# wtaylor17/ImageCFGen-Pytorch

Hardware: AMD Instinct MI355X
Metric: ALI training images/sec (E+G+D step), MorphoMNIST bs=512/GPU (higher is better)
Workload: dtype f32; 1 GPU; image_scms/mnist.py ALI iteration (EG step + 2 D steps + diagnostics), MorphoMNIST 28x28x1 synthetic, bs=512/GPU, fp32 MFMA, mode=stepper+hipgraph; global_batch=512, parallelism=dp1

## Files before the change

imagecfgen-pytorch_amd/ali_hip/_lib.py:

```python
import ctypes
import os
from ctypes import POINTER, Structure, c_char_p, c_double, c_float, c_int32, c_int64, c_size_t, c_uint64, c_void_p

_HERE = os.path.dirname(os.path.abspath(__file__))
LIB_PATH = os.path.join(_HERE, "libali_hip.so")


class AliHipUnavailable(RuntimeError):
    pass


class AliConvGeom(Structure):
    _fields_ = [(n, c_int32) for n in ("B", "H", "W", "C", "P", "Q", "K", "R", "S", "stride", "pad")]


class AliEpilogue(Structure):
    _fields_ = [("bias", c_void_p), ("act", c_int32), ("slope", c_float), ("mask", c_void_p), ("mask_ld", c_int32),
                ("dact_y", c_void_p), ("dact", c_int32), ("dslope", c_float),
                ("bn_part", c_void_p), ("bn_mode", c_int32), ("bn_groups", c_int32), ("bn_stat_mask", c_void_p),
                ("bn_mask_ld", c_int32), ("bn_x", c_void_p), ("bn_mean", c_void_p), ("bn_invstd", c_void_p),
                ("bn_mask_in", c_void_p), ("bn_mask_pre", c_void_p), ("mfma_f16", c_int32),
                ("in16", c_void_p), ("w16", c_void_p), ("out16", c_void_p),
                ("tile_order", c_void_p), ("tile_order_n", c_int32), ("in_ld", c_int32), ("out_ld", c_int32),
                ("in_ch_live", c_int32), ("bn_slots", c_int32), ("dact_y16", c_void_p)]
# ... 183 lines not shown
    "ali_add_i64_multi": (c_int32, [c_int32, POINTER(c_void_p), POINTER(c_int64), c_void_p]),
    "ali_assemble_planes": (c_int32, [c_void_p, c_void_p, POINTER(c_void_p), c_int32, c_void_p, c_int32, c_void_p,
                                      c_int32, c_int32, c_int32, c_int32, c_void_p, c_int32, c_void_p]),
    "ali_spect_post": (c_int32, [c_void_p, c_int32, c_int32, c_int32, c_void_p, c_void_p, c_float, c_void_p, c_void_p]),
    "ali_plane_table_grad": (c_int32, [c_void_p, c_int32, c_int32, c_void_p, c_int32, c_int32, c_void_p, c_int32, c_int32,
                                       c_int32, c_int32, c_int32, c_int32, c_void_p, c_void_p, c_void_p]),
    "ali_col2im": (c_int32, [c_void_p, c_int32, c_void_p, c_void_p] + [c_int32] * 12 + [c_float, c_void_p]),
    "ali_tconv_scatter_ok": (c_int32, [c_int32] * 5),
    "ali_tconv_scatter_wgrad_ws": (c_int64, [c_int32] * 7),
    "ali_tconv_scatter_wgrad": (c_int32, [c_void_p, c_void_p, c_int32, c_void_p, c_int64, c_int64] + [c_int32] * 10
                                + [c_void_p, c_size_t, c_void_p]),
    "ali_tconv_scatter": (c_int32, [c_void_p] * 4 + [c_int32] * 13 + [c_float, c_void_p]),
    "ali_tconv_scatter_plan": (c_int32, [c_int32] * 13 + [POINTER(c_int64)]),
    "ali_tconv1_fwd": (c_int32, [c_void_p, c_void_p, c_void_p, c_void_p] + [c_int32] * 9 + [c_float, c_void_p, c_int32,
                                                                                            c_void_p]),
    "ali_tconv1_dgrad": (c_int32, [c_void_p, c_int32, c_void_p, c_void_p, c_int32, c_float, c_void_p] + [c_int32] * 7
                         + [c_void_p]),
    "ali_tconv1_wgrad": (c_int32, [c_void_p, c_void_p, c_int32, c_int32, c_void_p, c_int64, c_int64, c_int64]
                         + [c_int32] * 7 + [c_void_p, c_size_t, c_void_p]),
    "ali_tconv1_route": (c_int32, [c_int32] * 9 + [c_size_t]),
    "ali_ssim_fwd": (c_int32, [c_void_p, c_void_p, c_int64, c_int32, c_int32, c_void_p, c_int32, c_float, c_float,
                               c_void_p, c_void_p, c_void_p, c_void_p, c_void_p, c_size_t, c_void_p]),
    "ali_ssim_bwd": (c_int32, [c_void_p, c_void_p, c_void_p, c_void_p, c_void_p, c_void_p, c_int64, c_int32, c_int32,
                               c_void_p, c_int32, c_void_p, c_void_p]),
    "ali_gl_init": (c_int32, [c_void_p, c_int32, c_int32, c_int32, c_int32, c_void_p, c_void_p, c_float, c_float, c_void_p,
                              c_void_p, c_int32, c_uint64, c_void_p, c_uint64, c_void_p, c_void_p, c_void_p]),
    "ali_gl_ola": (c_int32, [c_void_p, c_void_p, c_int32, c_int32, c_int32, c_int32, c_int32, c_int32, c_int64, c_int32,
                             c_void_p, c_int32, c_void_p, c_void_p]),
    "ali_gl_phase": (c_int32, [c_void_p, c_void_p, c_void_p, c_float, c_int64, c_int32, c_void_p, c_void_p]),
    "ali_gl_check": (c_int32, [c_int32, c_int32, c_int32, c_int32, c_int64]),
    "ali_last_error": (c_char_p, []),
    "ali_head_fwd": (c_int32, [c_void_p, c_int32, c_void_p, c_void_p, c_void_p, c_int32, c_int32, c_void_p]),
    "ali_head_wgrad": (c_int32, [c_void_p, c_int32, c_void_p, c_void_p, c_void_p, c_int32, c_int32, c_void_p]),
    "ali_copy_multi": (c_int32, [c_int32, POINTER(c_void_p), POINTER(c_void_p), POINTER(c_int64), c_void_p]),
    "ali_version": (c_int32, []),
    "ali_reload_tuning": (None, []),
}

_lib = None
_load_error = None


def load():
    global _lib, _load_error
    if _lib is not None:
        return _lib
    if not os.path.exists(LIB_PATH):
        _load_error = f"{LIB_PATH} not found: build it with `python __graft_entry__.py build` (hipcc, gfx950)"
        raise AliHipUnavailable(_load_error)
    try:
        lib = ctypes.CDLL(LIB_PATH)
    except OSError as e:
        _load_error = f"cannot load {LIB_PATH}: {e}"
        raise AliHipUnavailable(_load_error)
    for name, (res, args) in SIGNATURES.items():
        fn = getattr(lib, name)
        fn.restype = res
        fn.argtypes = args
    _lib = lib
    return lib


def check(rc, what):
    if rc != 0:
        msg = load().ali_last_error()
        raise RuntimeError(f"{what} failed (rc={rc}): {msg.decode() if msg else ''}")
# ... 1 lines not shown
```

imagecfgen-pytorch_amd/ali_hip/chain.py:

```python
import weakref
from collections import namedtuple
from typing import List, Optional

import torch
import torch.nn as nn

from . import dropout as _dropout
from . import ops
from .ops import ACT_LEAKY, ACT_NONE, ACT_TANH


def _pad4(c: int) -> int:
    return (c + 3) // 4 * 4


class Stage:
    __slots__ = ("kind", "mod", "act", "slope", "pre", "pattern", "has_drop", "drop_p", "bn", "unflat", "index", "hw")

    def __init__(self, kind, mod, pre, index):
        self.kind, self.mod, self.pre, self.index = kind, mod, pre, index
        self.act, self.slope, self.unflat = ACT_NONE, 0.0, None
        self.hw = None
        self.pattern = [k for k, _ in pre]
        self.has_drop = "drop" in self.pattern
# ... 603 lines not shown
        if st.kind == "flat":
            resolve_flat(st, (B, H, W, Cp), c_log)
        sv.in_shape, sv.out_shape = (B, H, W, Cp), _out_shape(st, B, H, W, Cp)
        sv.geom, sv.route = _geom(st, sv.in_shape, sv.out_shape), route(st, sv.in_shape, c_log)
        sv.mask = folded if folded is not None else early
        if sv.mask is None and st.has_drop and training:
            sv.mask = _dropout.next_mask(B, c_log, st.drop_p, cur.device, Cp, lane=lane)
        sv.t = _pre_ops(st, sv, bn_fwd and (bn_fwd[0], bn_fwd[3]), folded is not None or (si == 0 and first_mask_applied),
                        groups)
        K = sv.out_shape[3]
        out_ld, jmask = 0, None
        if nxt is None and join is not None:
            joint, joff, jm = join
            if sv.out_shape[1:3] != (1, 1) or joint.shape[0] != B or not join_ok(plan):
                raise ValueError("chain_forward(join=...): the last stage must be a plain conv GEMM onto a 1x1 map")
            out_ld = joint.shape[1]
            sv.y = joint[:, joff:joff + K].unflatten(1, (1, 1, K))
            jmask = None if jm is None else jm[:, joff:joff + K]
        else:
            sv.y = (alloc(("y", si), sv.out_shape) if alloc is not None
                    else torch.empty(sv.out_shape, dtype=torch.float32, device=cur.device))
        folded, early, bn_fwd = _for_next_stage(nxt, sv, groups, lane) if nxt is not None else (None, None, None)
        yield from _launch_fwd(plan, st, sv, folded, bn_fwd, out_ld, jmask, alloc)
        if save:
            saved.append(sv)
        cur, c_log = sv.y, K
    return cur, saved


def wgrad_geoms(plan: ChainPlan, saved):
    return [sv.geom for sv in saved if sv.route.wgrad[0] != "tconv1"]


def _param_grads(st: Stage, sv, g_pre, ld: int, grads, grad_dst, fold):
    m, g = st.mod, sv.geom
    B, H, W, Cp = sv.in_shape
    _, P, Q, K = sv.out_shape
    c_in = sv.c_log
    path, db_path = sv.route.wgrad if fold is None else sv.route.wgrad_fold
    fused_db = None
    if db_path == "unflat":
        Cc, hh, ww = st.unflat
        db = ops.colsum(B, hh * ww * Cc, hh * ww * Cc, g_pre).reshape(hh * ww, Cc).t().reshape(-1)
        grads[id(m.bias)] = grad_dst[id(m.bias)].copy_(db) if id(m.bias) in grad_dst else db
    elif db_path == "fused":
        fused_db = grad_dst.get(id(m.bias))
        if fused_db is None:
            fused_db = torch.empty(K, dtype=torch.float32, device=g_pre.device)
        grads[id(m.bias)] = fused_db
    elif db_path == "colsum":
        grads[id(m.bias)] = ops.colsum(B * P * Q, K, K, g_pre, out=grad_dst.get(id(m.bias)))
    dw = grads[id(m.weight)] = grad_dst[id(m.weight)] if id(m.weight) in grad_dst else torch.empty_like(m.weight)
    if path == "flat_repack":
        O, I, T = m.out_features, m.in_features, H * W
        tmp = torch.empty(O, I, device=dw.device)
        ops.conv_bwd_weight(g, sv.t, g_pre, tmp, I, O, I, 1, 0)
        ops.pack_weights(tmp, dw, O, I // T, T, T, I, 1, I // T)
        return
    if st.kind == "flat":
        ops.conv_bwd_weight(g, sv.t, g_pre, dw, c_in, K, dw.stride(0), H * W, 1, db=fused_db, dy_ld=ld, defer=fold)
        return
    R, S = m.kernel_size if st.kind != "linear" else (1, 1)
    if path == "convT_scatter" and sv.t.is_contiguous() and g_pre.is_contiguous() and dw.stride(2) == S * dw.stride(3):
        if ops.tconv_scatter_wgrad(sv.t, g_pre, 1, dw, dw.stride(0), dw.stride(3), B, H, W, Cp, P, Q, R, S, m.stride[0],
                                   m.padding[0]) is not None:
            return
    if path == "head":
        ops.head_wgrad(sv.t.reshape(B, Cp)[:, :c_in], g_pre.reshape(B), dw.reshape(-1), db=fused_db)
    elif path == "first_direct":
        ops.tconv1_wgrad(g_pre, sv.t, Cp, c_in, dw, c_in * R * S, 1, R * S, B, P, Q, K, R, S, m.padding[0])
    elif path == "conv":
        ops.conv_bwd_weight(g, sv.t, g_pre, dw, c_in, K, dw.stride(0), dw.stride(1), dw.stride(3), db=fused_db,
                            dy_ld=ld, defer=fold)
    elif path == "tconv1":
        ops.tconv1_wgrad(sv.t, g_pre, 1, 1, dw, R * S, 1, 0, B, H, W, Cp, R, S, m.padding[0])
    elif path in ("convT", "convT_scatter"):
        ops.conv_bwd_weight(g, g_pre, sv.t, dw, K, c_in, dw.stride(0), dw.stride(1), dw.stride(3), defer=fold)
    elif path == "linear":
        ops.conv_bwd_weight(g, sv.t, g_pre, dw, m.in_features, m.out_features, m.in_features, 1, 0, defer=fold)
    else:
        (O, I), (Cc, hh, ww) = m.weight.shape, st.unflat
        tmp = torch.empty(O, I, device=dw.device)
        ops.conv_bwd_weight(g, sv.t, g_pre, tmp, I, O, I, 1, 0)
        ops.pack_weights(tmp, dw, Cc, hh * ww, I, I, I, Cc * I, 1)


def _plane_grads(plan: ChainPlan, st: Stage, sv, g_pre, gx_planes):
    m, NP = st.mod, len(gx_planes)
    B, H, W, Cp = sv.in_shape
    _, P, Q, K = sv.out_shape
    R, S = m.kernel_size
    form = sv.route.planes
    if form is None or (form == "scatter" and not (1 <= NP <= 8 and NP * R * S <= 128)):
        return None
    planes = torch.empty(B, H, W, NP, dtype=torch.float32, device=g_pre.device)
    if form == "direct":
        wd = plan.packed(st, "dgrad", Cp)
        for j, c in enumerate(gx_planes):
            ops.tconv1_fwd(g_pre, wd[c], None, planes[..., j], B, P, Q, K, R, S, m.padding[0], NP, ACT_NONE, 0.0,
                           rowscale=None if sv.mask is None else sv.mask[:, c])
        return planes
    wd = plan.packed(st, ("scatter_dgrad", tuple(gx_planes)), Cp)
    if ops.tconv_scatter_ok(K, NP, R, S, m.stride[0]) and g_pre.is_contiguous():
        ops.tconv_scatter(g_pre, wd, None, planes, B, P, Q, K, H, W, NP, NP, R, S, m.stride[0], m.padding[0])
    else:
        contrib = torch.empty(B, P, Q, NP * R * S, dtype=torch.float32, device=g_pre.device)
        ops.conv_fwd(ops.geom(B, P, Q, K, P, Q, NP * R * S, 1, 1, 1, 0), g_pre, wd, contrib, ops.epilogue())
        yield
        ops.col2im(contrib, NP * R * S, None, planes, B, P, Q, H, W, NP, NP, R, S, m.stride[0], m.padding[0])
    if sv.mask is not None:
        cols = torch.cat([sv.mask[:, c:c + 1] for c in gx_planes], dim=1)
        planes = planes * cols.reshape(B, 1, 1, -1)
    return planes


def _data_grad(plan: ChainPlan, st: Stage, sv, g_pre, ld: int, pact, pslope, want: bool, need_params: bool, grads,
               grad_dst):
    m, g, bn, rt = st.mod, sv.geom, sv.bn, sv.route
    B, H, W, Cp = sv.in_shape
    dact_y = sv.x_in if pact != ACT_NONE else None
    gt = torch.empty(sv.in_shape, dtype=torch.float32, device=g_pre.device)
    bn_red = None
    if bn is None:
        ep = ops.epilogue(mask=sv.mask, dact_y=dact_y, dact=pact, dslope=pslope)
    else:
        mask_in = sv.mask if sv.pattern == ["drop", "bn"] else None
        mask_pre = sv.mask if sv.pattern == ["bn", "drop"] else None
        slots = ops.conv_mtiles(g, 0 if rt.dgrad == "convT" else 1)[0] if rt.bn_reduce else 0
        if slots > 0:
            bn_red = (torch.empty(2 * Cp * slots, dtype=torch.float32, device=g_pre.device), slots)
            ep = ops.epilogue(bn_bwd=(bn_red[0], sv.x_in, sv.bn_stats[0], sv.bn_stats[1], mask_in, mask_pre, slots))
        else:
            ep = ops.epilogue()
    if rt.dgrad == "tconv1" and bn is None and sv.mask is None:
        ops.tconv1_dgrad(g_pre, 1, plan.packed(st, "fwd", Cp), dact_y, pact, pslope, gt, B, H, W, Cp, m.kernel_size[0],
                         m.kernel_size[1], m.padding[0])
    elif st.kind == "convT":
        ops.conv_fwd(g, g_pre, plan.packed(st, "dgrad", Cp), gt, ep, live=(None, sv.c_log))
        yield
    else:
        wc = H * W * Cp if rt.dgrad == "flat_gemm" else Cp
        ops.conv_bwd_data(g, g_pre, plan.packed(st, "dgrad", wc), gt, ep, in_ld=ld,
                          live=(wc if rt.dgrad == "flat_gemm" else sv.c_log, None))
        yield
    if bn is None:
        return gt
    use_batch = sv.training or bn.running_mean is None
    slope = pslope if pact == ACT_LEAKY else -1.0
    out = dict(want_gx=want, out_dgamma=grad_dst.get(id(bn.weight)) if need_params else None,
               out_dbeta=grad_dst.get(id(bn.bias)) if need_params else None)
    if bn_red is not None:
        dgam, dbet, gprev = ops.bn_bwd_from_partials(bn_red[0], bn_red[1], sv.x_in, gt, mask_in, mask_pre, sv.bn_stats,
                                                     bn.weight.detach(), B, H * W, Cp, use_batch, slope, **out)
    else:
        dgam, dbet, gprev = ops.bn_bwd(sv.x_in, gt, mask_in, mask_pre, sv.bn_stats, bn.weight.detach(), B, H * W, Cp,
                                       use_batch, slope, **out)
    if need_params:
        grads[id(bn.weight)], grads[id(bn.bias)] = dgam, dbet
    if pact == ACT_TANH and gprev is not None:
        gprev = ops.act_bwd(gprev, sv.x_in, ACT_TANH, 0.0)
    return gprev


def chain_backward_gen(plan: ChainPlan, saved, gy: torch.Tensor, c_log_in: int, need_gx: bool, need_params: bool = True,
                       grad_dst=None, gx_planes=None, gy_ld: int = 0, gy_pre: bool = False, in_act=None, fold=None):
    grads = {}
    grad_dst = grad_dst or {}
    n = len(plan.stages)
    last = plan.stages[-1]
    assert saved[0].c_log == c_log_in, "chain_backward: c_log_in differs from the forward pass's"
    if gy_ld:
        if not (gy_pre or last.act == ACT_NONE) or not join_ok(plan):
            raise ValueError("chain_backward(gy_ld=...): needs join_ok(plan) and a pre-activation gradient")
        g_pre = gy
    else:
        gy = gy.contiguous()
        g_pre = gy if (gy_pre or last.act == ACT_NONE) else ops.act_bwd(gy, saved[-1].y, last.act, last.slope)
    for i in range(n - 1, -1, -1):
        st, sv = plan.stages[i], saved[i]
        assert not isinstance(sv.bn_stats, list), "grouped forward state: backpropagate slice_saved(saved, g, groups)"
        ld = gy_ld if i == n - 1 else 0
        if need_params:
            _param_grads(st, sv, g_pre, ld, grads, grad_dst, fold)
        if i > 0:
            g_pre = yield from _data_grad(plan, st, sv, g_pre, ld, plan.stages[i - 1].act, plan.stages[i - 1].slope, True,
                                          need_params, grads, grad_dst)
    gx = (yield from _plane_grads(plan, st, sv, g_pre, gx_planes)) if gx_planes is not None else None
    if gx is None and (need_gx or sv.bn is not None):
        gx = yield from _data_grad(plan, st, sv, g_pre, ld, *(in_act or (ACT_NONE, 0.0)), need_gx, need_params, grads,
                                   grad_dst)
    return gx, grads


def _plain_stack(plan: ChainPlan, what: str):
    for st in plan.stages:
        if st.pre or st.kind not in ("conv", "flat") or st.act not in (ACT_NONE, ACT_LEAKY):
            raise NotImplementedError(f"ali_hip.chain.{what}: needs a stack of Conv2d / Flatten + Linear stages with "
                                      f"LeakyReLU or no activation and nothing in front of them (stage {st.index}: "
                                      f"{st.kind}, pre-ops {st.pattern}, activation {st.act})")


def saved_rows(saved, lo: int, hi: int):
    out = []
    for sv in saved:
        assert sv.bn is None and sv.bn_stats is None, "saved_rows: BatchNorm statistics couple the rows of a batch"
        s2 = _Saved()
        s2.x_in, s2.t, s2.y = sv.x_in[lo:hi], sv.t[lo:hi], sv.y[lo:hi]
        s2.mask = None if sv.mask is None else sv.mask[lo:hi]
        s2.bn, s2.bn_stats, s2.pattern, s2.training, s2.route, s2.c_log = None, None, sv.pattern, sv.training, sv.route, sv.c_log
        s2.in_shape, s2.out_shape = (hi - lo,) + tuple(sv.in_shape[1:]), (hi - lo,) + tuple(sv.out_shape[1:])
        g = sv.geom
        s2.geom = ops.geom(hi - lo, g.H, g.W, g.C, g.P, g.Q, g.K, g.R, g.S, g.stride, g.pad)
        out.append(s2)
    return out


def chain_backward_keep_gen(plan: ChainPlan, saved, gy: torch.Tensor, c_log_in: int, need_gx: bool = True,
                            gx_planes=None, first_rows=None):
    _plain_stack(plan, "chain_backward_keep")
# ... 120 lines not shown
```

imagecfgen-pytorch_amd/ali_hip/ops.py:

```python
import collections
import ctypes
from ctypes import byref, c_void_p

import numpy as np
import torch

from . import _lib
from ._lib import ACT_LEAKY, ACT_NONE, ACT_TANH, AliConvGeom, AliEpilogue

_WS = {}
_WS_BYTES = 256 << 20


def set_workspace_bytes(n: int):
    global _WS_BYTES
    _WS_BYTES = int(n)
    _WS.clear()


def workspace(device, slot: int = 0) -> torch.Tensor:
    key = (device.type, device.index if device.index is not None else torch.cuda.current_device(), slot)
    ws = _WS.get(key)
    if ws is None or ws.numel() < _WS_BYTES:
        ws = torch.zeros(_WS_BYTES, dtype=torch.uint8, device=device)
# ... 670 lines not shown
def _flush_packs():
    jobs = _PACK_BATCH
    if not jobs:
        return
    _launch_packs(jobs)
    jobs.clear()


def pack_weights(src, dst, N, T, C, Cpad, s_n, s_tap, s_c):
    _chk(src, "src"), _chk(dst, "dst")
    if _PACK_BATCH is not None:
        if any(j[1].data_ptr() == src.data_ptr() for j in _PACK_BATCH):
            _flush_packs()
        _PACK_BATCH.append((src, dst, N, T, C, Cpad, s_n, s_tap, s_c))
        return dst
    _launch_packs([(src, dst, N, T, C, Cpad, s_n, s_tap, s_c)])
    return dst


def head_fwd(x2d, w, bias, y):
    B, C = x2d.shape
    _lib.check(_lib.load().ali_head_fwd(_ptr(x2d), x2d.stride(0), _chk(w, "w"), _opt(bias, "bias"), _chk(y, "y"), B, C,
                                        _stream()), "ali_head_fwd")
    return y


def head_wgrad(x2d, g, dw, db=None):
    B, C = x2d.shape
    _lib.check(_lib.load().ali_head_wgrad(_ptr(x2d), x2d.stride(0), _chk(g, "g"), _chk(dw, "dw"), _opt(db, "db"), B, C,
                                          _stream()), "ali_head_wgrad")
    return dw


def copy_multi(pairs):
    fast = []
    for dst, src in pairs:
        if (dst.is_cuda and src.is_cuda and dst.device == src.device and dst.dtype == src.dtype and dst.shape == src.shape
                and dst.is_contiguous() and src.is_contiguous() and dst.element_size() % 4 == 0 and dst.numel() > 0):
            fast.append((dst, src))
        else:
            dst.copy_(src)
    if fast:
        n = len(fast)
        srcs = (c_void_p * n)(*[s_.data_ptr() for _, s_ in fast])
        dsts = (c_void_p * n)(*[d_.data_ptr() for d_, _ in fast])
        sizes = (ctypes.c_int64 * n)(*[d_.numel() * d_.element_size() for d_, _ in fast])
        _lib.check(_lib.load().ali_copy_multi(n, srcs, dsts, sizes, _stream()), "ali_copy_multi")


def act_bwd(gy, y, act, slope, out=None):
    lib = _lib.load()
    out = torch.empty_like(gy) if out is None else out
    _lib.check(lib.ali_act_bwd(_chk(gy, "gy"), _chk(y, "y"), _chk(out), gy.numel(), act, slope, _stream()),
               "ali_act_bwd")
    return out


def colsum(x2d_rows, C, ld, x, out=None):
    lib = _lib.load()
    ws = workspace(x.device)
    out = torch.empty(C, dtype=torch.float32, device=x.device) if out is None else out
    _lib.check(lib.ali_colsum(_chk(x, "x"), x2d_rows, C, ld, _chk(out), c_void_p(ws.data_ptr()), ws.numel(),
                              _stream()), "ali_colsum")
    return out


# ... 1376 lines not shown
```

imagecfgen-pytorch_amd/ali_hip/step.py:

```python
from collections import namedtuple
from typing import Dict

import torch

from . import dp
from . import dropout as _dropout
from . import ops
from . import source as _source
from . import ssim
from . import chain as _chain
from .chain import (chain_backward, chain_backward_gen, chain_forward, chain_forward_gen, drive, get_plan,
                    run_parallel, slice_saved)
from .graphs import GraphCache, _Graphed
from .trainer import FlatGroup, Stepper, load_module_state_, module_state_cpu


class MnistFamily:
    name = "mnist"
    hw = (28, 28)

    def __init__(self, E, G, D):
        self.e_tables = [E.digit_embedding[0].weight]
        self.d_tables = [D.digit_embedding[0].weight]
        self.g_tables = [G.digit_embedding.weight]
# ... 409 lines not shown
        self._refresh_d()

    def _phase_eg(self, cx):
        self._eg_grads(cx)
        if self.dist:
            dp.allreduce_sum_(self.opt_eg.grad, self.pg)
        self._apply_eg()

    def _phase_d_real(self, cx):
        self._d_real_pre(cx)
        self._d_real_rest(cx)
        if self.dist:
            dp.allreduce_sum_(self.opt_d.grad, self.pg)
        self._apply_d()

    def _phase_d_fake(self, cx):
        self._d_fake_pre(cx)
        self._d_fake_rest(cx)
        if self.dist:
            dp.allreduce_sum_(self.opt_d.grad, self.pg)
        self._apply_d()

    def _d_real_input(self, cx):
        cx["x0d"], cx["n_log"], masked = self._d_planes(cx["images"], cx["idx"], cx["cont"])
        return cx["x0d"], cx["n_log"], masked

    def _d_real_pre(self, cx):
        x0d, n_log, masked = self._d_real_input(cx)
        cx["dx_pre"] = self._dx_forward(x0d, n_log, True, x_masked=masked)

    def _d_real_all(self, cx):
        x0d, n_log, masked = self._d_real_input(cx)
        x0e, _ = self._planes(cx["images"], cx["idx"], cx["cont"], self.family.e_tables)
        cx["dx_pre"], (cx["ex_pre"], _) = run_parallel(self._dx_forward_gen(x0d, n_log, True, x_masked=masked),
                                                       chain_forward_gen(self.pE, x0e, True, n_log, False))
        self._d_real_rest(cx)

    def _d_real_rest(self, cx):
        fam, images, idx, cont = self.family, cx["images"], cx["idx"], cx["cont"]
        x0d, n_log = cx["x0d"], cx["n_log"]
        ex = cx.pop("ex_pre", None)
        if ex is None:
            x0e, _ = self._planes(images, idx, cont, fam.e_tables)
            ex, _ = chain_forward(self.pE, x0e, True, n_log, False)
        dx_pre, join = cx.pop("dx_pre")
        d_valid, sD = self._d_forward(x0d, n_log, ex, True, dx_pre=dx_pre, join=join)
        l, gl = ops.bce_logits(d_valid, 1.0, self.loss_scale)
        cx["out"]["loss_d_real"] = l[0]
        g_x0, _ = self._d_backward(sD, gl, True, True, False, planes=self._emb_planes)
        self._plane_grads(g_x0, idx, fam.d_tables, self.opt_d.grad_views)
        cx["ex"] = ex

    def _d_fake_pre(self, cx):
        gin, g_log = self._g_input(cx["zin"], cx["onehots"], cx["cont"])
        cx["gz"], _ = chain_forward(self.pG, gin, True, g_log, False)

    def _d_fake_rest(self, cx):
        fam, idx, cont, zin = self.family, cx["idx"], cx["cont"], cx["zin"]
        x0f, _, masked = self._d_planes(cx["gz"], idx, cont)
        d_fake, sD = self._d_forward(x0f, cx["n_log"], zin, True, x_masked=masked)
        l, gl = ops.bce_logits(d_fake, 0.0, self.loss_scale)
        cx["out"]["loss_d_fake"] = l[0]
        g_x0, _ = self._d_backward(sD, gl, True, True, False, planes=self._emb_planes)
        self._plane_grads(g_x0, idx, fam.d_tables, self.opt_d.grad_views)

    def _phase_scores(self, cx, average_bn=True):
        fam, images, idx, cont, zin = self.family, cx["images"], cx["idx"], cx["cont"], cx["zin"]
        logits, _ = self._d_forward_pair(cx["gz"], zin, images, cx["ex"].reshape(zin.shape), idx, cont, False)
        s3 = ops.bce_logits_pair(logits, cx["B"], 0.0, 0.0, 1.0, want_grad=False)[0]
        cx["out"]["dg"], cx["out"]["de"] = s3[1], s3[2]
        _dropout.end_iteration()
        _chain.flush_batch_counts(extra=[(self.iter_t, 1)])
        if self.dist and average_bn:
            dp.average_buffers_(self.bn_buffers, self.pg)

    def _pipelined(self, do_eg):
        return self.pipeline_reduce and do_eg and (self.dist or self.segmented)

    def _segments(self, do_eg, ahead=False):
        segs = []
        if not (self.dist or self.segmented):
            if do_eg:
                segs.append((lambda cx: self._eg_grads(cx), self.opt_eg, False))
                segs.append((lambda cx: (self._apply_eg(), self._d_real_all(cx)), self.opt_d, True))
            else:
                segs.append((lambda cx: self._d_real_all(cx), self.opt_d, False))
# ... 315 lines not shown
```

imagecfgen-pytorch_amd/csrc/elementwise.hip:

```cpp
#include "ali_common.h"
#include <algorithm>
#include <string.h>

namespace ali {

constexpr int kEwBlock = 256;
static inline int ew_grid(long long n, int per_thread = 1) {
  long long b = (n + (long long)kEwBlock * per_thread - 1) / ((long long)kEwBlock * per_thread);
  if (b > 2048) b = 2048;
  if (b < 1) b = 1;
  return (int)b;
}

__global__ void pack_weights_kernel(const float* __restrict__ src, float* __restrict__ dst, int N, int T, int C,
                                    int Cpad, long long s_n, long long s_tap, long long s_c) {
  const long long total = (long long)N * T * Cpad;
  long long i = (long long)blockIdx.x * blockDim.x + threadIdx.x;
  const long long step = (long long)gridDim.x * blockDim.x;
  for (; i < total; i += step) {
    const int c = (int)(i % Cpad);
    const long long nt = i / Cpad;
    const int tp = (int)(nt % T);
    const long long n = nt / T;
    dst[i] = c < C ? src[n * s_n + tp * s_tap + c * s_c] : 0.f;
// ... 915 lines not shown
  const int cl = threadIdx.x & 31, rl = threadIdx.x >> 5;
  const int c = blockIdx.x * 32 + cl;
  float acc[8];
#pragma unroll
  for (int u = 0; u < 8; ++u) acc[u] = 0.f;
  float s0 = 0.f;
  const bool sum_g = blockIdx.x == 0 && cl == 0 && db != nullptr;
  if (c < C || sum_g) {
    const int cc = c < C ? c : 0;
    for (int b0 = rl; b0 < B; b0 += 64) {
      float gv[8], xv[8];
#pragma unroll
      for (int u = 0; u < 8; ++u) {
        const int b = b0 + 8 * u;
        gv[u] = b < B ? g[b] : 0.f;
        xv[u] = b < B ? x[(long long)b * ld + cc] : 0.f;
      }
#pragma unroll
      for (int u = 0; u < 8; ++u) { acc[u] += gv[u] * xv[u]; s0 += gv[u]; }
    }
  }
  red[rl][cl] = ((acc[0] + acc[1]) + (acc[2] + acc[3])) + ((acc[4] + acc[5]) + (acc[6] + acc[7]));
  if (cl == 0) red[rl][32] = s0;
  __syncthreads();
  if (rl == 0) {
    float v = red[0][cl], sg = red[0][32];
#pragma unroll
    for (int r = 1; r < 8; ++r) { v += red[r][cl]; sg += red[r][32]; }
    if (c < C) dw[c] = v;
    if (sum_g) db[0] = sg;
  }
}

constexpr int kCopyJobs = 8;
struct CopyJobs { int n; const unsigned* src[kCopyJobs]; unsigned* dst[kCopyJobs]; long long words[kCopyJobs]; int blk0[kCopyJobs + 1]; };
__global__ void __launch_bounds__(256) copy_multi_kernel(const CopyJobs jobs) {
  int k = 0;
#pragma unroll 1
  for (int i = 1; i < jobs.n; ++i)
    if ((int)blockIdx.x >= jobs.blk0[i]) k = i;
  const long long i0 = ((long long)(blockIdx.x - jobs.blk0[k]) * 256 + threadIdx.x) * 4;
  const long long n = jobs.words[k];
  const unsigned* s = jobs.src[k];
  unsigned* d = jobs.dst[k];
  if (i0 + 4 <= n && ((((unsigned long long)s) | ((unsigned long long)d)) & 15ull) == 0) {
    *reinterpret_cast<uint4*>(d + i0) = *reinterpret_cast<const uint4*>(s + i0);
  } else {
    for (long long i = i0; i < n && i < i0 + 4; ++i) d[i] = s[i];
  }
}

__global__ void __launch_bounds__(kEwBlock)
normal_fill_kernel(uint64_t seed, const long long* __restrict__ dev_counter, uint64_t offset, float* __restrict__ out,
                   long long n, int head) {
  const uint64_t key = latent_key(rng_base_key(seed, dev_counter));
  const long long nvec = (n - head) >> 2, tail0 = head + 4 * nvec;
  const long long step = (long long)gridDim.x * blockDim.x;
  for (long long v = (long long)blockIdx.x * blockDim.x + threadIdx.x; v < nvec; v += step) {
    const long long i0 = head + 4 * v;
    const uint64_t g = offset + (uint64_t)i0;
    f32x4 r;
    if ((g & 1) == 0) {
      float c0, s0, c1, s1;
      normal_pair(key, g >> 1, c0, s0);
      normal_pair(key, (g >> 1) + 1, c1, s1);
      r = f32x4{c0, s0, c1, s1};
// ... 112 lines not shown
      blk += (long long)J.batch * J.ti * J.tj;
    } else if (J.tiled) {
      J.Ipad = J.Cpad;
      J.out_j = J.Ipad;
      J.ti = (J.Ipad + 31) / 32; J.tj = (J.J + 31) / 32;
      blk += (long long)J.batch * J.ti * J.tj;
    } else {
      long long nb = ((long long)J.N * J.T * J.Cpad + kEwBlock * 4 - 1) / (kEwBlock * 4);
      if (nb > 256) nb = 256;
      if (nb < 1) nb = 1;
      blk += nb;
    }
    if (blk >= (1LL << 31)) { set_error("ali_pack_weights_multi: too many tiles"); return ALI_ERR_BAD_ARG; }
  }
  jobs.n = n_jobs;
  hipLaunchKernelGGL(pack_weights_multi_kernel, dim3((unsigned)blk), dim3(kEwBlock), 0, ST(stream), jobs);
  return check_launch("pack_weights_multi_kernel");
}

extern "C" int ali_head_fwd(const float* x, int32_t ld, const float* w, const float* bias, float* y, int32_t B, int32_t C,
                            ali_stream_t stream) {
  if (!x || !w || !y || B <= 0 || C <= 0 || (C % 4) || ld < C || (ld % 4)) { set_error("ali_head_fwd: bad argument"); return ALI_ERR_BAD_ARG; }
  hipLaunchKernelGGL(head_fwd_kernel, dim3((B + 3) / 4), dim3(256), 0, ST(stream), x, ld, w, bias, y, B, C);
  return check_launch("head_fwd_kernel");
}

extern "C" int ali_head_wgrad(const float* x, int32_t ld, const float* g, float* dw, float* db, int32_t B, int32_t C,
                              ali_stream_t stream) {
  if (!x || !g || !dw || B <= 0 || C <= 0 || ld < C) { set_error("ali_head_wgrad: bad argument"); return ALI_ERR_BAD_ARG; }
  hipLaunchKernelGGL(head_wgrad_kernel, dim3((C + 31) / 32), dim3(256), 0, ST(stream), x, ld, g, dw, db, B, C);
  return check_launch("head_wgrad_kernel");
}

extern "C" int ali_copy_multi(int32_t n, const void* const* src, void* const* dst, const int64_t* bytes, ali_stream_t stream) {
  if (n < 0 || (n > 0 && (!src || !dst || !bytes))) { set_error("ali_copy_multi: bad argument"); return ALI_ERR_BAD_ARG; }
  for (int j0 = 0; j0 < n; j0 += kCopyJobs) {
    CopyJobs cj;
    memset(&cj, 0, sizeof(cj));
    int blocks = 0;
    for (int i = j0; i < n && i < j0 + kCopyJobs; ++i) {
      if (!src[i] || !dst[i] || bytes[i] < 0 || (bytes[i] & 3) || ((unsigned long long)src[i] & 3) || ((unsigned long long)dst[i] & 3)) {
        set_error("ali_copy_multi: job %d: pointers and sizes must be multiples of 4 bytes", i);
        return ALI_ERR_BAD_ARG;
      }
      const int k = cj.n++;
      cj.src[k] = reinterpret_cast<const unsigned*>(src[i]);
      cj.dst[k] = reinterpret_cast<unsigned*>(dst[i]);
      cj.words[k] = bytes[i] / 4;
      cj.blk0[k] = blocks;
      const long long nb = (cj.words[k] + 1023) / 1024;
      if (blocks + nb > (1 << 30)) { set_error("ali_copy_multi: too large"); return ALI_ERR_BAD_ARG; }
      blocks += (int)nb;
    }
    cj.blk0[cj.n] = blocks;
    if (blocks > 0) hipLaunchKernelGGL(copy_multi_kernel, dim3(blocks), dim3(256), 0, ST(stream), cj);
    int rc = check_launch("copy_multi_kernel");
    if (rc) return rc;
  }
  return ALI_OK;
}

extern "C" int ali_act_bwd(const float* gy, const float* y, float* gpre, int64_t n, int32_t act, float slope,
                           ali_stream_t stream) {
  if (!gy || !y || !gpre || n < 0) { set_error("ali_act_bwd: bad argument"); return ALI_ERR_BAD_ARG; }
  if (n == 0) return ALI_OK;
  EwPlan pl;
// ... 411 lines not shown
```

include/ali_hip.h:

```cpp
#ifndef ALI_HIP_H
#define ALI_HIP_H

#include <stddef.h>
#include <stdint.h>

#ifdef __cplusplus
extern "C" {
#endif

typedef void* ali_stream_t;
#define ALI_WS_RESERVED 4096

typedef enum {
  ALI_OK = 0,
  ALI_ERR_BAD_ARG = -1,
  ALI_ERR_WORKSPACE = -2,
  ALI_ERR_LAUNCH = -3
} AliStatus;

typedef enum { ALI_ACT_NONE = 0, ALI_ACT_LEAKY = 1, ALI_ACT_TANH = 2 } AliAct;

typedef struct {
  int32_t B, H, W, C;
  int32_t P, Q, K;
// ... 382 lines not shown
#define ALI_TS_OP_FWD 0
#define ALI_TS_OP_WGRAD 1
int32_t ali_tconv_scatter_plan(int32_t op, int32_t B, int32_t H, int32_t W, int32_t C, int32_t Hout, int32_t Wout,
                               int32_t NC, int32_t ostride, int32_t R, int32_t S, int32_t stride, int32_t pad,
                               int64_t* plan);

int ali_spect_post(const float* y, int32_t B, int32_t T, int32_t F, const float* mean, const float* std, float clip_k,
                   float* out, ali_stream_t stream);

#define ALI_SSIM_MAX_WIN 25
int ali_ssim_fwd(const float* X, const float* Y, int64_t planes, int32_t H, int32_t W, const float* win,
                 int32_t win_size, float C1, float C2, float* ssim_pc, float* mA, float* mB, float* mC, void* ws,
                 size_t ws_bytes, ali_stream_t stream);
int ali_ssim_bwd(const float* X, const float* Y, const float* mA, const float* mB, const float* mC, const float* gpc,
                 int64_t planes, int32_t H, int32_t W, const float* win, int32_t win_size, float* dY,
                 ali_stream_t stream);

typedef enum { ALI_GL_SRC_IMAGE = 0, ALI_GL_SRC_LOG = 1, ALI_GL_SRC_SPEC = 2 } AliGlSource;
int ali_gl_init(const float* src, int32_t B, int32_t F, int32_t T, int32_t mode, const float* mean, const float* std,
                float stds_kept, float power, const float* a0_re, const float* a0_im, int32_t rand_init, uint64_t seed,
                const int64_t* dev_counter, uint64_t offset, float* mag, float* X, ali_stream_t stream);
int ali_gl_ola(const float* fr, const float* renv, int32_t n_renv, int32_t B, int32_t T, int32_t n_fft, int32_t win,
               int32_t hop, int64_t length, int32_t final_wave, float* out, int32_t frames_per_block, int64_t* advance,
               ali_stream_t stream);
int ali_gl_phase(const float* Y, const float* tprev, const float* mag, float m, int64_t rows, int32_t F, float* X,
                 ali_stream_t stream);
int32_t ali_gl_check(int32_t n_fft, int32_t win, int32_t hop, int32_t T, int64_t length);

const char* ali_last_error(void);
int ali_head_fwd(const float* x, int32_t ld, const float* w, const float* bias, float* y, int32_t B, int32_t C,
                 ali_stream_t stream);
int ali_head_wgrad(const float* x, int32_t ld, const float* g, float* dw, float* db, int32_t B, int32_t C,
                   ali_stream_t stream);
int ali_copy_multi(int32_t n, const void* const* src, void* const* dst, const int64_t* bytes, ali_stream_t stream);
int ali_version(void);
void ali_reload_tuning(void);

#ifdef __cplusplus
}
#endif
#endif
```

Baseline: 84000 images/s.

## Fuse discriminator head backward with wgrad and run G forward alongside D-real chains

Adds a head_bwd kernel that computes the data gradient through the scalar discriminator head, including activation grad and dropout mask, and can also produce the head weight and bias grads in the same pass. It reduces partial sums through workspace with a last-block counter. The head wgrad is deferred into this fused kernel, replacing a separate wgrad launch plus the generic conv dgrad path. Separately, the generator forward is launched in parallel with the D-real and encoder forward chains, so G(z) is ready before the fake pass. The trade-off is more kernel code, cross-block atomic handshakes, and a changed execution order.

Result: faster. 85000 images/s, median of 6 (+1.2%).

```diff
diff --git a/imagecfgen-pytorch_amd/ali_hip/_lib.py b/imagecfgen-pytorch_amd/ali_hip/_lib.py
--- a/imagecfgen-pytorch_amd/ali_hip/_lib.py
+++ b/imagecfgen-pytorch_amd/ali_hip/_lib.py
@@ -239,6 +239,8 @@
     "ali_last_error": (c_char_p, []),
     "ali_head_fwd": (c_int32, [c_void_p, c_int32, c_void_p, c_void_p, c_void_p, c_int32, c_int32, c_void_p]),
     "ali_head_wgrad": (c_int32, [c_void_p, c_int32, c_void_p, c_void_p, c_void_p, c_int32, c_int32, c_void_p]),
+    "ali_head_bwd": (c_int32, [c_void_p, c_void_p, c_void_p, c_int32, c_float, c_void_p, c_int32, c_void_p, c_void_p,
+                               c_int32, c_void_p, c_void_p, c_int32, c_int32, c_void_p, c_size_t, c_void_p]),
     "ali_copy_multi": (c_int32, [c_int32, POINTER(c_void_p), POINTER(c_void_p), POINTER(c_int64), c_void_p]),
     "ali_version": (c_int32, []),
     "ali_reload_tuning": (None, []),
diff --git a/imagecfgen-pytorch_amd/ali_hip/chain.py b/imagecfgen-pytorch_amd/ali_hip/chain.py
--- a/imagecfgen-pytorch_amd/ali_hip/chain.py
+++ b/imagecfgen-pytorch_amd/ali_hip/chain.py
@@ -659,7 +659,14 @@
     return [sv.geom for sv in saved if sv.route.wgrad[0] != "tconv1"]
 
 
-def _param_grads(st: Stage, sv, g_pre, ld: int, grads, grad_dst, fold):
+def _head_bwd_ok(st: Stage, sv, ld: int) -> bool:
+    return (sv.route.fwd == "head" and sv.route.wgrad[0] == "head" and sv.bn is None and ld == 0
+            and not ops._PRECISION["f16"]
+            and sv.c_log == sv.in_shape[3] and sv.t.is_contiguous() and sv.x_in.is_contiguous()
+            and (sv.mask is None or sv.mask.stride(1) == 1) and not ops.switched_off("ALI_NO_HEAD_BWD"))
+
+
+def _param_grads(st: Stage, sv, g_pre, ld: int, grads, grad_dst, fold, head_later: bool = False):
     m, g = st.mod, sv.geom
     B, H, W, Cp = sv.in_shape
     _, P, Q, K = sv.out_shape
@@ -692,6 +699,8 @@
         if ops.tconv_scatter_wgrad(sv.t, g_pre, 1, dw, dw.stride(0), dw.stride(3), B, H, W, Cp, P, Q, R, S, m.stride[0],
                                    m.padding[0]) is not None:
             return
+    if path == "head" and head_later:
+        return dw.reshape(-1), fused_db
     if path == "head":
         ops.head_wgrad(sv.t.reshape(B, Cp)[:, :c_in], g_pre.reshape(B), dw.reshape(-1), db=fused_db)
     elif path == "first_direct":
@@ -742,11 +751,17 @@
 
 
 def _data_grad(plan: ChainPlan, st: Stage, sv, g_pre, ld: int, pact, pslope, want: bool, need_params: bool, grads,
-               grad_dst):
+               grad_dst, head_pg=None):
     m, g, bn, rt = st.mod, sv.geom, sv.bn, sv.route
     B, H, W, Cp = sv.in_shape
     dact_y = sv.x_in if pact != ACT_NONE else None
     gt = torch.empty(sv.in_shape, dtype=torch.float32, device=g_pre.device)
+    if _head_bwd_ok(st, sv, ld):
+        dw, db = head_pg if head_pg is not None else (None, None)
+        ops.head_bwd(g_pre.reshape(B), plan.packed(st, "fwd", Cp).reshape(-1), dact_y, pact, pslope, sv.mask,
+                     gt.reshape(B, Cp), sv.t.reshape(B, Cp), dw, db)
+        yield
+        return gt
     bn_red = None
     if bn is None:
         ep = ops.epilogue(mask=sv.mask, dact_y=dact_y, dact=pact, dslope=pslope)
@@ -807,11 +822,13 @@
         st, sv = plan.stages[i], saved[i]
         assert not isinstance(sv.bn_stats, list), "grouped forward state: backpropagate slice_saved(saved, g, groups)"
         ld = gy_ld if i == n - 1 else 0
+        head_pg = None
         if need_params:
-            _param_grads(st, sv, g_pre, ld, grads, grad_dst, fold)
+            head_pg = _param_grads(st, sv, g_pre, ld, grads, grad_dst, fold,
+                                   head_later=i > 0 and _head_bwd_ok(st, sv, ld))
         if i > 0:
             g_pre = yield from _data_grad(plan, st, sv, g_pre, ld, plan.stages[i - 1].act, plan.stages[i - 1].slope, True,
-                                          need_params, grads, grad_dst)
+                                          need_params, grads, grad_dst, head_pg)
     gx = (yield from _plane_grads(plan, st, sv, g_pre, gx_planes)) if gx_planes is not None else None
     if gx is None and (need_gx or sv.bn is not None):
         gx = yield from _data_grad(plan, st, sv, g_pre, ld, *(in_act or (ACT_NONE, 0.0)), need_gx, need_params, grads,
diff --git a/imagecfgen-pytorch_amd/ali_hip/ops.py b/imagecfgen-pytorch_amd/ali_hip/ops.py
--- a/imagecfgen-pytorch_amd/ali_hip/ops.py
+++ b/imagecfgen-pytorch_amd/ali_hip/ops.py
@@ -726,6 +726,29 @@
     return dw
 
 
+def switched_off(name: str) -> bool:
+    import os
+    return os.environ.get(name, "0") not in ("", "0")
+
+
+def head_bwd(gl, w, y_prev, dact, dslope, mask, g, x2d=None, dw=None, db=None):
+    B, C = g.shape
+    if gl.numel() != B or w.numel() != C or (y_prev is not None and y_prev.numel() != B * C):
+        raise ValueError("head_bwd: operand shapes do not match g [B, C]")
+    if dw is not None and (x2d is None or tuple(x2d.shape) != (B, C) or x2d.stride(1) != 1 or dw.numel() != C):
+        raise ValueError("head_bwd: dw needs x2d [B, C] with unit column stride and C weights")
+    if mask is not None and (mask.shape[0] != B or mask.shape[1] < C or mask.stride(1) != 1):
+        raise ValueError("head_bwd: mask must be [B, >= C] with unit column stride")
+    ws = workspace(g.device)
+    _lib.check(_lib.load().ali_head_bwd(_chk(gl, "gl"), _chk(w, "w"), _opt(y_prev, "y_prev"), dact, dslope,
+                                        None if mask is None else _ptr(mask), 0 if mask is None else mask.stride(0),
+                                        _chk(g, "g"),
+                                        None if dw is None else _ptr(x2d), 0 if dw is None else x2d.stride(0),
+                                        _opt(dw, "dw"), _opt(db, "db"), B, C, c_void_p(ws.data_ptr()), ws.numel(),
+                                        _stream()), "ali_head_bwd")
+    return g
+
+
 def copy_multi(pairs):
     fast = []
     for dst, src in pairs:
diff --git a/imagecfgen-pytorch_amd/ali_hip/step.py b/imagecfgen-pytorch_amd/ali_hip/step.py
--- a/imagecfgen-pytorch_amd/ali_hip/step.py
+++ b/imagecfgen-pytorch_amd/ali_hip/step.py
@@ -465,8 +465,14 @@
     def _d_real_all(self, cx):
         x0d, n_log, masked = self._d_real_input(cx)
         x0e, _ = self._planes(cx["images"], cx["idx"], cx["cont"], self.family.e_tables)
-        cx["dx_pre"], (cx["ex_pre"], _) = run_parallel(self._dx_forward_gen(x0d, n_log, True, x_masked=masked),
-                                                       chain_forward_gen(self.pE, x0e, True, n_log, False))
+        gens = [self._dx_forward_gen(x0d, n_log, True, x_masked=masked), chain_forward_gen(self.pE, x0e, True, n_log, False)]
+        if not ops.switched_off("ALI_NO_GZ_CHAIN"):
+            gin, g_log = self._g_input(cx["zin"], cx["onehots"], cx["cont"])
+            gens.append(chain_forward_gen(self.pG, gin, True, g_log, False))
+        res = run_parallel(*gens)
+        cx["dx_pre"], cx["ex_pre"] = res[0], res[1][0]
+        if len(res) > 2:
+            cx["gz"] = res[2][0]
         self._d_real_rest(cx)
 
     def _d_real_rest(self, cx):
@@ -485,6 +491,8 @@
         cx["ex"] = ex
 
     def _d_fake_pre(self, cx):
+        if "gz" in cx:
+            return
         gin, g_log = self._g_input(cx["zin"], cx["onehots"], cx["cont"])
         cx["gz"], _ = chain_forward(self.pG, gin, True, g_log, False)
 
diff --git a/imagecfgen-pytorch_amd/csrc/elementwise.hip b/imagecfgen-pytorch_amd/csrc/elementwise.hip
--- a/imagecfgen-pytorch_amd/csrc/elementwise.hip
+++ b/imagecfgen-pytorch_amd/csrc/elementwise.hip
@@ -971,6 +971,99 @@
   }
 }
 
+__device__ __forceinline__ float head_bwd_value(float gv, float wv, bool has_mask, float mk, bool has_y, float yv, int dact,
+                                                float dslope) {
+  float v = gv * wv + 0.f;
+  if (has_mask) v *= mk;
+  if (has_y) v *= act_grad_from_output(yv, dact, dslope);
+  return v;
+}
+__global__ void __launch_bounds__(256) head_bwd_kernel(const float* __restrict__ gl, const float* __restrict__ w,
+                                                       const float* __restrict__ yprev, int dact, float dslope,
+                                                       const float* __restrict__ mask, int mask_ld, float* __restrict__ g,
+                                                       int B, int C) {
+  const int cl = threadIdx.x & 31, rl = threadIdx.x >> 5;
+  const int c = blockIdx.x * 32 + cl;
+  if (c >= C) return;
+  const float wv = w[c];
+  const int b0 = (int)blockIdx.y * 64 + rl;
+  float gv[8], yv[8], mk[8];
+#pragma unroll
+  for (int u = 0; u < 8; ++u) {
+    const int b = b0 + 8 * u;
+    const bool ok = b < B;
+    gv[u] = ok ? gl[b] : 0.f;
+    yv[u] = (ok && yprev) ? yprev[(long long)b * C + c] : 0.f;
+    mk[u] = (ok && mask) ? mask[(long long)b * mask_ld + c] : 1.f;
+  }
+#pragma unroll
+  for (int u = 0; u < 8; ++u) {
+    const int b = b0 + 8 * u;
+    if (b < B) g[(long long)b * C + c] = head_bwd_value(gv[u], wv, mask != nullptr, mk[u], yprev != nullptr, yv[u], dact, dslope);
+  }
+}
+
+__global__ void __launch_bounds__(256) head_bwd_wg_kernel(const float* __restrict__ gl, const float* __restrict__ w,
+                                                          const float* __restrict__ yprev, int dact, float dslope,
+                                                          const float* __restrict__ mask, int mask_ld, float* __restrict__ g,
+                                                          const float* __restrict__ x, int ld, float* __restrict__ dw,
+                                                          float* __restrict__ db, int B, int C, float* part, int* ctr) {
+  __shared__ float red[8][33];
+  __shared__ int s_last;
+  const int cl = threadIdx.x & 31, u = threadIdx.x >> 5, rl = blockIdx.y;
+  const int c = blockIdx.x * 32 + cl;
+  const bool live = c < C;
+  const bool sum_g = blockIdx.x == 0 && threadIdx.x == 0 && db != nullptr;
+  const bool x_is_y = x == yprev && ld == C;
+  float acc = 0.f;
+  if (live) {
+    const float wv = w[c];
+#pragma unroll 8
+    for (int b = rl + 8 * u; b < B; b += 64) {
+      const float gv = gl[b], xv = x[(long long)b * ld + c];
+      const float yv = x_is_y ? xv : yprev ? yprev[(long long)b * C + c] : 0.f;
+      const float mk = mask ? mask[(long long)b * mask_ld + c] : 1.f;
+      g[(long long)b * C + c] = head_bwd_value(gv, wv, mask != nullptr, mk, yprev != nullptr, yv, dact, dslope);
+      acc += gv * xv;
+    }
+  }
+  red[u][cl] = acc;
+  float s0 = 0.f;
+  if (sum_g) {
+    for (int b0 = rl; b0 < B; b0 += 64)
+#pragma unroll
+      for (int k = 0; k < 8; ++k)
+        if (b0 + 8 * k < B) s0 += gl[b0 + 8 * k];
+  }
+  __syncthreads();
+  if (u == 0) {
+    const float v = ((red[0][cl] + red[1][cl]) + (red[2][cl] + red[3][cl])) + ((red[4][cl] + red[5][cl]) + (red[6][cl] + red[7][cl]));
+    if (live) __hip_atomic_store(part + (long long)rl * C + c, v, __ATOMIC_RELAXED, __HIP_MEMORY_SCOPE_AGENT);
+    if (sum_g) __hip_atomic_store(part + (long long)8 * C + rl, s0, __ATOMIC_RELAXED, __HIP_MEMORY_SCOPE_AGENT);
+    asm volatile("s_waitcnt vmcnt(0)" ::: "memory");
+  }
+  __syncthreads();
+  if (threadIdx.x == 0) {
+    const int arrived = __hip_atomic_fetch_add(ctr + blockIdx.x, 1, __ATOMIC_RELAXED, __HIP_MEMORY_SCOPE_AGENT);
+    s_last = arrived == 7;
+    if (s_last) __hip_atomic_store(ctr + blockIdx.x, 0, __ATOMIC_RELAXED, __HIP_MEMORY_SCOPE_AGENT);
+  }
+  __syncthreads();
+  if (!s_last || u != 0) return;
+  if (live) {
+    float v = __hip_atomic_load(part + c, __ATOMIC_RELAXED, __HIP_MEMORY_SCOPE_AGENT);
+#pragma unroll
+    for (int r = 1; r < 8; ++r) v += __hip_atomic_load(part + (long long)r * C + c, __ATOMIC_RELAXED, __HIP_MEMORY_SCOPE_AGENT);
+    dw[c] = v;
+  }
+  if (sum_g) {
+    float sg = __hip_atomic_load(part + (long long)8 * C, __ATOMIC_RELAXED, __HIP_MEMORY_SCOPE_AGENT);
+#pragma unroll
+    for (int r = 1; r < 8; ++r) sg += __hip_atomic_load(part + (long long)8 * C + r, __ATOMIC_RELAXED, __HIP_MEMORY_SCOPE_AGENT);
+    db[0] = sg;
+  }
+}
+
 constexpr int kCopyJobs = 8;
 struct CopyJobs { int n; const unsigned* src[kCopyJobs]; unsigned* dst[kCopyJobs]; long long words[kCopyJobs]; int blk0[kCopyJobs + 1]; };
 __global__ void __launch_bounds__(256) copy_multi_kernel(const CopyJobs jobs) {
@@ -1149,6 +1242,31 @@
   return check_launch("head_wgrad_kernel");
 }
 
+extern "C" int ali_head_bwd(const float* gl, const float* w, const float* y_prev, int32_t dact, float dslope,
+                            const float* mask, int32_t mask_ld, float* g, const float* x, int32_t ld, float* dw, float* db,
+                            int32_t B, int32_t C, void* ws, size_t ws_bytes, ali_stream_t stream) {
+  if (!gl || !w || !g || B <= 0 || C <= 0 || (mask && mask_ld < C) || (dw && (!x || ld < C)) || (db && !dw) ||
+      (dact != ALI_ACT_NONE && !y_prev)) {
+    set_error("ali_head_bwd: bad argument");
+    return ALI_ERR_BAD_ARG;
+  }
+  if (dact == ALI_ACT_NONE) y_prev = nullptr;
+  const int cb = (C + 31) / 32;
+  if (!dw) {
+    hipLaunchKernelGGL(head_bwd_kernel, dim3(cb, (B + 63) / 64), dim3(256), 0, ST(stream), gl, w, y_prev, dact, dslope,
+                       mask, mask_ld, g, B, C);
+    return check_launch("head_bwd_kernel");
+  }
+  const size_t need = ((size_t)8 * C + 8) * sizeof(float);
+  if (!ws || ws_payload_bytes(ws_bytes) < need || cb > (int)(kWsReserved / sizeof(int))) {
+    set_error("ali_head_bwd: workspace too small (%zu bytes behind the reserved head needed)", need);
+    return ALI_ERR_WORKSPACE;
+  }
+  hipLaunchKernelGGL(head_bwd_wg_kernel, dim3(cb, 8), dim3(256), 0, ST(stream), gl, w, y_prev, dact, dslope, mask, mask_ld,
+                     g, x, ld, dw, db, B, C, reinterpret_cast<float*>(ws_payload(ws)), reinterpret_cast<int*>(ws));
+  return check_launch("head_bwd_wg_kernel");
+}
+
 extern "C" int ali_copy_multi(int32_t n, const void* const* src, void* const* dst, const int64_t* bytes, ali_stream_t stream) {
   if (n < 0 || (n > 0 && (!src || !dst || !bytes))) { set_error("ali_copy_multi: bad argument"); return ALI_ERR_BAD_ARG; }
   for (int j0 = 0; j0 < n; j0 += kCopyJobs) {
diff --git a/include/ali_hip.h b/include/ali_hip.h
--- a/include/ali_hip.h
+++ b/include/ali_hip.h
@@ -438,6 +438,9 @@
                  ali_stream_t stream);
 int ali_head_wgrad(const float* x, int32_t ld, const float* g, float* dw, float* db, int32_t B, int32_t C,
                    ali_stream_t stream);
+int ali_head_bwd(const float* gl, const float* w, const float* y_prev, int32_t dact, float dslope, const float* mask,
+                 int32_t mask_ld, float* g, const float* x, int32_t ld, float* dw, float* db, int32_t B, int32_t C,
+                 void* ws, size_t ws_bytes, ali_stream_t stream);
 int ali_copy_multi(int32_t n, const void* const* src, void* const* dst, const int64_t* bytes, ali_stream_t stream);
 int ali_version(void);
 void ali_reload_tuning(void);
```
